# DoumanAsh/compu

Hardware: AMD Instinct MI355X
Metric: decompressed GB/s (whole node), batched 64 KiB DEFLATE blocks; % HBM peak (higher is better)
Workload: dtype u8

## Files before the change

compu_amd/csrc/inflate_unit.h:

```cpp
#pragma once
#include "chip_internal.h"
#include "wave_checksums.h"

namespace chip {

typedef uint32_t u32x2 __attribute__((ext_vector_type(2)));
typedef uint32_t u32x4 __attribute__((ext_vector_type(4)));
typedef u32x4 u32x4_u __attribute__((aligned(1)));
typedef u32x4 u32x4_a4 __attribute__((aligned(4)));
template <typename T>
__device__ __forceinline__ GAS T *rdfirst_gptr(T *p)
{
    return (GAS T *)rdfirst_ptr(p);
}

#ifndef CHIP_PHASE_FN
#define CHIP_PHASE_FN __attribute__((always_inline))
#endif

#ifdef CHIP_STATS
#define STAT_DECL unsigned long long st_[24] = {0}; unsigned long long st_t0_ = 0
#define STAT_T0() (st_t0_ = __builtin_readcyclecounter())
#define STAT_ACC(i) do { unsigned long long n_ = __builtin_readcyclecounter(); st_[i] += n_ - st_t0_; st_t0_ = n_; } while (0)
#define STAT_ADD(i, v) (st_[i] += (unsigned long long)(v))
#define STAT_PARAM , unsigned long long *st_, unsigned long long &st_t0_
#define STAT_ARG , st_, st_t0_
#else
#define STAT_DECL
#define STAT_T0()
#define STAT_ACC(i)
#define STAT_ADD(i, v)
#define STAT_PARAM
#define STAT_ARG
#endif

enum : uint32_t { K_LIT = 0, K_LEN = 1, K_EOB = 2, K_BAD = 3 };
__device__ __forceinline__ constexpr uint32_t mk_entry(uint32_t cl, uint32_t eb, uint32_t kind, uint32_t base)
{
    return cl | (eb << 4) | (kind << 8) | (base << 16);
}

constexpr int LIT_ROOT = 9;
constexpr int DIST_ROOT = 8;
constexpr int CL_ROOT = 7;

constexpr uint32_t F_HALT = 1u << 15, F_INV = 1u << 26, F_LEN = 1u << 31;
constexpr uint32_t D_BAD = 1u << 10, D_LONG = 1u << 15;
static_assert(15 - LIT_ROOT < 8 && 15 - DIST_ROOT < 8, "a root entry's index bit count leaves its bits [4:3] clear");
static_assert((2u << (15 - DIST_ROOT)) - 2u < 256u, "the distance sub-tables fit the 256 units that a root entry's offset spans");

__device__ __forceinline__ uint32_t make_final(uint32_t sym, uint32_t len)
{
    if (sym < 256) return len | (len << 10) | (sym << 16);
    if (sym == 256) return len | (len << 10) | F_HALT;
    if (sym >= 286) return len | (len << 10) | F_HALT | F_INV;
    const uint32_t s = sym - 257;
    uint32_t eb = 0, base = 3 + s;
    if (s == 28) base = 258;
    else if (s >= 8) {
        eb = (s >> 2) - 1;
        base = 3 + ((4 + (s & 3)) << eb);
    }
    return len | (eb << 5) | ((len + eb) << 10) | ((512u | base) << 16) | F_LEN;
}
__device__ __forceinline__ uint32_t make_dist16(uint32_t sym, uint32_t len)
{
    if (sym >= 30) return len | D_BAD;
    if (sym < 4) return len | (sym << 8);
    return len | (((sym >> 1) - 1) << 4) | ((2 + (sym & 1)) << 8);
}

#ifndef CHIP_S_BITS
#define CHIP_S_BITS 320
#define CHIP_XT_BITS 1536
#define CHIP_XT_BITS_FIXED 3072
#define CHIP_ROW_TOKENS 256
#endif
constexpr uint32_t S_BITS = CHIP_S_BITS;
constexpr uint32_t XT_BITS = CHIP_XT_BITS;
#ifndef CHIP_XT_BITS_FIXED
#define CHIP_XT_BITS_FIXED CHIP_XT_BITS
#endif
constexpr uint32_t XT_BITS_FIXED = CHIP_XT_BITS_FIXED;
constexpr uint32_t ROW_TOKENS = CHIP_ROW_TOKENS;
static_assert(S_BITS % 32 == 0 && ROW_TOKENS % 4 == 0 && 64 * ROW_TOKENS < 65536, "geometry");
constexpr uint32_t SEG_WORDS = S_BITS / 32 + 1;
constexpr uint32_t SEG_SHIFT = 24;
constexpr uint32_t SEG_MAGIC = ((1u << SEG_SHIFT) + S_BITS - 1) / S_BITS;
constexpr bool seg_magic_ok()
{
    for (uint32_t x = 0; x < 64u * S_BITS + 4096u; x++)
        if (((x * SEG_MAGIC) >> SEG_SHIFT) != x / S_BITS) return false;
    return true;
}
static_assert(seg_magic_ok() && (64u * S_BITS + 4096u) * (uint64_t)SEG_MAGIC < (1ull << 32), "segment index by multiplication");
constexpr uint32_t WIN_DW = (31 + 64 * S_BITS + 48 + 96 + 31) / 32 + 3;
constexpr uint32_t HDR_IN_DW = 192;

constexpr size_t ROWS_WORDS = (size_t)64 * ROW_TOKENS;
static_assert(64ull * ROW_TOKENS * 258 < (1ull << 32), "count_tokens() sums a super-round's output lengths in 32 bits");
__device__ __forceinline__ uint32_t row_base(uint32_t l) { return (l >> 3) * (8u * ROW_TOKENS) + (l & 7u) * 4u; }
__device__ __forceinline__ uint32_t row_word(uint32_t k) { return k + (k >> 2) * 28u; }

__device__ __forceinline__ uint32_t tok_olen(uint32_t t) { return (t & 512u) ? t & 0x1ffu : 1u + (t >> 31); }

struct HuffMeta {
    uint32_t limit15[16];
    uint32_t offs[16];
    uint32_t maxlen;
};

#ifndef CHIP_CHUNK_BYTES
#define CHIP_CHUNK_BYTES 2560
#endif
#ifndef CHIP_COPY_LANE_MAX
#define CHIP_COPY_LANE_MAX 32
#endif
constexpr uint32_t CHUNK_BYTES = CHIP_CHUNK_BYTES;
constexpr uint32_t COPY_LANE_MAX = CHIP_COPY_LANE_MAX;
constexpr uint32_t MQ_CAP = 128;
constexpr uint32_t IMG_WORDS = CHUNK_BYTES / 4 + 8;
constexpr uint32_t TOK_RING = 4;
static_assert(CHUNK_BYTES % 4 == 0 && CHUNK_BYTES >= 1024 && COPY_LANE_MAX % 16 == 0 && IMG_WORDS % 2 == 0, "geometry");

constexpr uint32_t FLUSH_BYTES = 4 * (IMG_WORDS + 2 * MQ_CAP + 64 * TOK_RING + 128 + 4);
constexpr uint32_t HDR_BYTES = 4 * HDR_IN_DW + 4 * (1 << CL_ROOT) + 80 + sizeof(HuffMeta) + 64 + 320 + 2 * 288 + 2 * 32 + 2 * sizeof(HuffMeta);
constexpr uint32_t PHASE_BYTES = 8 * WIN_DW > FLUSH_BYTES ? (8 * WIN_DW > HDR_BYTES ? 8 * WIN_DW : HDR_BYTES) : (FLUSH_BYTES > HDR_BYTES ? FLUSH_BYTES : HDR_BYTES);
#ifndef CHIP_LDS_BYTES
#define CHIP_LDS_BYTES 8960
#endif
constexpr uint32_t POOL_WORDS = (CHIP_LDS_BYTES - 2 * 512 - 2 * 256 - PHASE_BYTES) / 4;
constexpr uint32_t POOL_U16 = 2 * POOL_WORDS;
constexpr uint32_t DIST_SUB_BYTES = 2 * (POOL_U16 - 256);

struct alignas(16) WaveLds {
    union {
        struct {
            uint32_t win[WIN_DW];
            uint32_t bm[WIN_DW];
        } w;
        struct {
            uint32_t inbuf[HDR_IN_DW];
            uint32_t cl_lut[1 << CL_ROOT];
            uint32_t cl_sorted[20];
            HuffMeta cl_h;
            uint32_t count[16];
            uint8_t lens[320];
            uint16_t lit_sorted[288];
            uint16_t dist_sorted[32];
            HuffMeta lit_h, dist_h;
        } hdr;
        struct {
            uint32_t out[IMG_WORDS];
            uint2 mq[MQ_CAP];
            uint32_t tok[64 * TOK_RING];
            uint32_t pk[128];
            uint32_t trash[4];
        } fl;
        uint32_t phase_words_[PHASE_BYTES / 4];
    };
    uint16_t lit_root[1 << LIT_ROOT];
    uint16_t dist_root[1 << DIST_ROOT];
    uint32_t pool[POOL_WORDS];
};
static_assert(sizeof(WaveLds) <= CHIP_LDS_BYTES, "the waves per CU that CHIP_LDS_BYTES stands for");
static_assert(POOL_WORDS >= 413 + 142, "the tables of any valid block fit");
#ifndef CHIP_EXP_ALLOW_SMALL_LDS
static_assert(sizeof(WaveLds) >= 2048 * 4, "wave_crc32 needs 8 KB");
#endif

__device__ __forceinline__ uint32_t canon_index(const HuffMeta &H, uint32_t x15, uint32_t &l)
{
    l = 1;
    if (x15 >= H.limit15[15]) return 0xffffffffu;
#pragma unroll
    for (int j = 1; j < 15; j++) l += (x15 >= H.limit15[j]) ? 1u : 0u;
    return H.offs[l] + ((x15 - H.limit15[l - 1]) >> (15 - l));
}

struct CanonLim {
    uint32_t lim[16];
};
__device__ __forceinline__ CanonLim canon_limits(const HuffMeta &H)
{
    CanonLim c;
#pragma unroll
    for (int j = 0; j < 16; j++) c.lim[j] = rdfirst(H.limit15[j]);
    return c;
}
template <int LO, int HI>
__device__ __forceinline__ uint32_t canon_index_in(const HuffMeta &H, const CanonLim &c, uint32_t x15, uint32_t &l)
{
    l = LO;
#pragma unroll
    for (int j = LO; j < HI; j++) l += (x15 >= c.lim[j]) ? 1u : 0u;
    return H.offs[l] + ((x15 - H.limit15[l - 1]) >> (15 - l));
}

template <typename SortedT, typename MakeT>
__device__ __forceinline__ int canon_prep(uint32_t *count, const uint8_t *lens, int n_, bool code_lengths, SortedT *sorted, HuffMeta &H, MakeT make)
{
    const uint32_t lane = lane_id();
    const int n = (int)rdfirst((uint32_t)n_);
    if (lane < 16) count[lane] = 0;
    WSYNC();
    for (int s = lane; s < n; s += 64) {
        uint32_t l = lens[s];
        if (l) atomicAdd(&count[l], 1u);
    }
    WSYNC();
    const uint32_t c = lane >= 1 && lane <= 15 ? count[lane] : 0u;
    const uint32_t cincl = wave_incl_scan(c);
    const uint32_t off = cincl - c;
    const uint32_t lim = wave_incl_scan(lane <= 15 ? c << (15u - (lane & 15u)) : 0u);
    const uint32_t present = (uint32_t)__ballot(c != 0);
    const uint32_t maxlen = present ? 31u - (uint32_t)__clz((int)present) : 0u;
    const bool over = __any(lane <= 15 && lim > 32768u);
    const int left = rdlane(lim, 15) < 32768u ? 1 : 0;
    uint32_t mynext = off;
    if (lane <= 15) {
        H.limit15[lane] = lim;
        H.offs[lane] = off;
    }
    if (lane == 0) H.maxlen = maxlen;
    WSYNC();
    if (maxlen == 0) return 1;
    if (over) return -1;
    if (left > 0 && (code_lengths || maxlen != 1)) return -1;
    for (int base = 0; base < n; base += 64) {
        int s = base + (int)lane;
        uint32_t l = s < n ? lens[s] : 0;
        for (uint32_t pm = present & 0xfffeu; pm; pm &= pm - 1u) {
            const uint32_t ll = (uint32_t)__builtin_ctz(pm);
            uint64_t m = __ballot(l == ll);
            uint32_t bp = rdlane(mynext, ll);
            if (l == ll) sorted[bp + __popcll(m & lanemask_lt())] = make((uint32_t)s, l);
            if (lane == ll) mynext += __popcll(m);
        }
    }
    WSYNC();
    return 0;
}

__device__ CHIP_PHASE_FN int build_cl_table(WaveLds &L)
{
    const uint32_t lane = lane_id();
    HuffMeta &H = L.hdr.cl_h;
    const int r = canon_prep(L.hdr.count, L.hdr.lens, 19, true, L.hdr.cl_sorted, H, [](uint32_t s, uint32_t l) { return mk_entry(l, 0, K_LIT, s); });
    if (r < 0) return -1;
    for (uint32_t idx = lane; idx < (1u << CL_ROOT); idx += 64) {
        uint32_t e = mk_entry(1, 0, K_LIT, 0);
        if (r == 0) {
            uint32_t l;
            const uint32_t ci = canon_index(H, __brev(idx) >> 17, l);
            e = ci == 0xffffffffu ? mk_entry(H.maxlen, 0, K_BAD, 0) : L.hdr.cl_sorted[ci];
        }
        L.hdr.cl_lut[idx] = e;
    }
    WSYNC();
    return 0;
}

__device__ CHIP_PHASE_FN int build_litlen(WaveLds &L, const uint8_t *lens, int n, uint32_t &used)
{
    const uint32_t lane = lane_id();
    HuffMeta &H = L.hdr.lit_h;
    uint16_t *const sorted = L.hdr.lit_sorted;
    const int r = canon_prep(L.hdr.count, lens, n, false, sorted, H, [](uint32_t s, uint32_t) { return (uint16_t)s; });
    if (r != 0) return -1;
    const CanonLim CL = canon_limits(H);
    const uint32_t lim_r = CL.lim[LIT_ROOT], top = CL.lim[15];
    const uint32_t nshort = rdfirst(H.offs[LIT_ROOT + 1 <= 15 ? LIT_ROOT + 1 : 15]);
    const uint32_t nsym = rdfirst(H.offs[15]) + rdfirst(L.hdr.count[15]);
    const uint32_t nfirst = rdfirst(H.maxlen) <= (uint32_t)LIT_ROOT ? nsym : nshort;
    if (nfirst + 1 > POOL_WORDS) return 1;
    for (uint32_t i = lane; i < nfirst; i += 64) {
        const uint32_t s = sorted[i];
        L.pool[i] = make_final(s, lens[s]);
    }
    const uint32_t bad_idx = nfirst;
    const uint32_t bad_e = rdfirst(H.maxlen) | (rdfirst(H.maxlen) << 10) | F_HALT | F_INV;
    if (lane == 0) L.pool[bad_idx] = bad_e;
    for (uint32_t idx = lane; idx < (1u << LIT_ROOT); idx += 64) {
        const uint32_t x15 = __brev(idx) >> 17;
        if (x15 >= top) L.lit_root[idx] = (uint16_t)(bad_idx << 5);
        else if (x15 < lim_r) {
            uint32_t l;
            L.lit_root[idx] = (uint16_t)(canon_index_in<1, LIT_ROOT>(H, CL, x15, l) << 5);
        }
    }
    used = nfirst + 1;
    if (top > lim_r) {
        constexpr uint32_t P = 1u << (15 - LIT_ROOT);
        const uint32_t np = (top - lim_r + P - 1) / P;
        for (uint32_t j0 = 0; j0 < np; j0 += 64) {
            const uint32_t j = j0 + lane;
            const bool have = j < np;
            const uint32_t xj = lim_r + j * P;
            uint32_t sb = 0;
            if (have) {
                uint32_t l;
                (void)canon_index_in<LIT_ROOT + 1, 15>(H, CL, xj + P < top ? xj + P - 1 : top - 1, l);
                sb = l - LIT_ROOT;
            }
            const uint32_t size = have ? (1u << sb) : 0u;
            const uint32_t incl = wave_incl_scan(size);
            const uint32_t off = used + incl - size;
            const uint32_t total = rdlane(incl, 63);
            if (used + total > POOL_WORDS) return 1;
            if (have) {
                for (uint32_t t = 0; t < size; t++) {
                    const uint32_t x15 = sb ? xj + ((__brev(t) >> (32 - sb)) << (15 - LIT_ROOT - sb)) : xj;
                    uint32_t l, e = bad_e;
                    if (x15 < top) {
                        const uint32_t s = sorted[canon_index_in<LIT_ROOT + 1, 15>(H, CL, x15, l)];
                        e = make_final(s, l);
                    }
                    L.pool[off + t] = e;
                }
                L.lit_root[__brev(xj >> (15 - LIT_ROOT)) >> (32 - LIT_ROOT)] = (uint16_t)((off << 5) | sb);
            }
            used += total;
        }
    }
    WSYNC();
    return 0;
}

__device__ CHIP_PHASE_FN int build_dist(WaveLds &L, const uint8_t *lens, int n, uint32_t used)
{
    const uint32_t lane = lane_id();
    HuffMeta &H = L.hdr.dist_h;
    uint16_t *const sorted = L.hdr.dist_sorted;
    const int r = canon_prep(L.hdr.count, lens, n, false, sorted, H, [](uint32_t s, uint32_t) { return (uint16_t)s; });
    if (r < 0) return -1;
    if (r == 1) {
        for (uint32_t idx = lane; idx < (1u << DIST_ROOT); idx += 64) L.dist_root[idx] = (uint16_t)(1u | D_BAD);
        WSYNC();
        return 0;
    }
    const CanonLim CL = canon_limits(H);
    const uint32_t lim_r = CL.lim[DIST_ROOT], top = CL.lim[15], maxlen = rdfirst(H.maxlen);
    uint16_t *const pool16 = (uint16_t *)L.pool;
    for (uint32_t idx = lane; idx < (1u << DIST_ROOT); idx += 64) {
        const uint32_t x15 = __brev(idx) >> 17;
        if (x15 >= top) L.dist_root[idx] = (uint16_t)(maxlen | D_BAD);
        else if (x15 < lim_r) {
            uint32_t l;
            const uint32_t s = sorted[canon_index_in<1, DIST_ROOT>(H, CL, x15, l)];
            L.dist_root[idx] = (uint16_t)make_dist16(s, l);
        }
    }
    if (top > lim_r) {
        constexpr uint32_t P = 1u << (15 - DIST_ROOT);
        const uint32_t np = (top - lim_r + P - 1) / P;
        uint32_t used16 = 0;
        for (uint32_t j0 = 0; j0 < np; j0 += 64) {
            const uint32_t j = j0 + lane;
            const bool have = j < np;
            const uint32_t xj = lim_r + j * P;
            uint32_t sb = 0;
            if (have) {
                uint32_t l;
                (void)canon_index_in<DIST_ROOT + 1, 15>(H, CL, xj + P < top ? xj + P - 1 : top - 1, l);
                sb = l - DIST_ROOT;
            }
            const uint32_t size = have ? (1u << sb) : 0u;
            const uint32_t incl = wave_incl_scan(size);
            const uint32_t total = rdlane(incl, 63);
            if (2 * used + used16 + total > POOL_U16) return 1;
            const uint32_t base16 = POOL_U16 - used16 - incl;
            if (have) {
                for (uint32_t t = 0; t < size; t++) {
                    const uint32_t x15 = sb ? xj + ((__brev(t) >> (32 - sb)) << (15 - DIST_ROOT - sb)) : xj;
                    uint32_t l, e = maxlen | D_BAD;
                    if (x15 < top) {
                        const uint32_t s = sorted[canon_index_in<DIST_ROOT + 1, 15>(H, CL, x15, l)];
                        e = make_dist16(s, l);
                    }
                    pool16[base16 + t] = (uint16_t)e;
                }
                L.dist_root[__brev(xj >> (15 - DIST_ROOT)) >> (32 - DIST_ROOT)] = (uint16_t)(D_LONG | sb | ((2u * base16 - DIST_SUB_BYTES) << 3));
            }
            used16 += total;
        }
    }
    WSYNC();
    return 0;
}
__device__ __forceinline__ uint32_t pool_at(const WaveLds &L, uint32_t r, uint32_t x)
{
    return *(const uint32_t *)((const uint8_t *)L.pool + ((r >> 3) + (__builtin_amdgcn_ubfe(x, LIT_ROOT, r) << 2)));
}
__device__ __forceinline__ uint32_t dist_sub_at(const WaveLds &L, uint32_t m, uint32_t x)
{
    return *(const uint16_t *)((const uint8_t *)L.pool + DIST_SUB_BYTES + (__builtin_amdgcn_ubfe(m, 3, 9) + (__builtin_amdgcn_ubfe(x, DIST_ROOT, m) << 1)));
}

struct InWin {
    const uint32_t *g32;
    uint32_t total_dw;
    uint32_t win0;
};


__device__ __forceinline__ void win_load(WaveLds &L, InWin &w, uint32_t dw_start)
{
    WSYNC();
    w.win0 = dw_start;
    constexpr uint32_t PER_LANE = (HDR_IN_DW + 63) / 64;
    uint32_t v[PER_LANE];
#pragma unroll
    for (uint32_t j = 0; j < PER_LANE; j++) {
        const uint32_t i = dw_start + 64u * j + lane_id();
        v[j] = i < w.total_dw ? w.g32[i] : 0u;
    }
#pragma unroll
    for (uint32_t j = 0; j < PER_LANE; j++) {
        const uint32_t k = 64u * j + lane_id();
        if (k < HDR_IN_DW) L.hdr.inbuf[k] = v[j];
    }
    WSYNC();
}

__device__ __forceinline__ void win_ensure(WaveLds &L, InWin &w, uint32_t pos, uint32_t span = 64)
{
    uint32_t d = pos >> 5;
    if (d < w.win0 || d + ((span + 62u) >> 5) + 1u > w.win0 + HDR_IN_DW) win_load(L, w, d);
}

__device__ __forceinline__ void win_bits(const WaveLds &L, const InWin &w, uint32_t pos, uint32_t &lo, uint32_t &hi)
{
    uint32_t D = (pos >> 5) - w.win0, sh = pos & 31;
    uint32_t d0 = L.hdr.inbuf[D], d1 = L.hdr.inbuf[D + 1], d2 = L.hdr.inbuf[D + 2];
    lo = __builtin_amdgcn_alignbit(d1, d0, sh);
    hi = __builtin_amdgcn_alignbit(d2, d1, sh);
}

__device__ __forceinline__ void win_bits_uniform(const WaveLds &L, const InWin &w, uint32_t pos, uint32_t &lo, uint32_t &hi)
{
    uint32_t l, h;
    win_bits(L, w, pos, l, h);
    lo = rdfirst(l);
    hi = rdfirst(h);
}

__device__ __forceinline__ uint32_t bfe(uint32_t v, uint32_t off, uint32_t width) { return __builtin_amdgcn_ubfe(v, off, width); }

__device__ int32_t parse_wrapper(LDS_AS uint32_t *tab, const uint8_t *gin, uint32_t avail, int32_t format, uint32_t &wrap, uint32_t &hdr)
{
    wrap = 0;
    hdr = 0;
    if (avail < 2) return CHIP_NEED_INPUT;
    const uint32_t b0 = gin[0], b1 = gin[1];
    const bool allow_gzip = format == CHIP_FMT_GZIP || format == CHIP_FMT_AUTO;
    const bool allow_zlib = format == CHIP_FMT_ZLIB || format == CHIP_FMT_AUTO;
    if (allow_gzip && b0 == 0x1f && b1 == 0x8b) {
        wrap = 2;
        if (avail < 4) return CHIP_NEED_INPUT;
        const uint32_t flg = gin[3];
        if (gin[2] != 8) return Z_DATA_ERROR;
        if (flg & 0xe0) return Z_DATA_ERROR;
        if (avail < 10) return CHIP_NEED_INPUT;
        uint32_t k = 10;
        if (flg & 4) {
            if (avail < k + 2) return CHIP_NEED_INPUT;
            uint32_t xlen = gin[k] | ((uint32_t)gin[k + 1] << 8);
            k += 2;
            if (avail - k < xlen) return CHIP_NEED_INPUT;
            k += xlen;
        }
        for (uint32_t bit = 8; bit <= 16; bit <<= 1) {
            if (!(flg & bit)) continue;
            for (;;) {
                uint32_t idx = k + lane_id();
                uint64_t z = __ballot(idx < avail && gin[idx] == 0);
                if (z) {
                    k += (uint32_t)__ffsll((long long)z);
                    break;
                }
                if (avail - k <= 64) return CHIP_NEED_INPUT;
                k += 64;
            }
        }
        if (flg & 2) {
            if (avail < k + 2) return CHIP_NEED_INPUT;
            uint32_t crc = wave_crc32(tab, gin, k);
            if ((crc & 0xffffu) != (gin[k] | ((uint32_t)gin[k + 1] << 8))) return Z_DATA_ERROR;
            k += 2;
        }
        hdr = k;
        return ST_RUNNING;
    }
    if (!allow_zlib) return Z_DATA_ERROR;
    if (((b0 << 8) | b1) % 31u) return Z_DATA_ERROR;
    if ((b0 & 15u) != 8) return Z_DATA_ERROR;
    if ((b0 >> 4) + 8 > 15) return Z_DATA_ERROR;
    wrap = 1;
    hdr = 2;
    if (b1 & 0x20) {
        if (avail < 6) return CHIP_NEED_INPUT;
        hdr = 6;
        return CHIP_NEED_DICT;
    }
    return ST_RUNNING;
}

struct __attribute__((packed)) U32u { uint32_t v; };
struct __attribute__((packed)) U16u { uint16_t v; };
struct __attribute__((packed)) U128u { uint32_t x, y, z, w; };
typedef LDS_AS uint8_t lds_u8;

__device__ void wave_copy_stored(uint8_t *gdst, const uint32_t *g32, uint32_t total_dw, uint32_t so, uint32_t n)
{
    const uint32_t lane = lane_id();
    const uint8_t *gsrc = (const uint8_t *)g32 + so;
    uint32_t head = (uint32_t)((16u - ((uintptr_t)gdst & 15u)) & 15u);
    if (head > n) head = n;
    if (lane < head) gdst[lane] = gsrc[lane];
    uint32_t done = head;
    const uint32_t body = (n - done) & ~15u;
    if (body) {
        uint4 *d16 = (uint4 *)(gdst + done);
        const U128u *s16 = (const U128u *)(gsrc + done);
        const uint32_t cnt = body >> 4;
        uint32_t i = lane;
#ifdef CHIP_STORED_NT_LD
#define CHIP_STORED_LD(p) __builtin_nontemporal_load(p)
#else
#define CHIP_STORED_LD(p) (*(p))
#endif
#ifndef CHIP_STORED_PLAIN_ST
#define CHIP_STORED_ST(v, p) __builtin_nontemporal_store(v, p)
#else
#define CHIP_STORED_ST(v, p) (*(p) = (v))
#endif
#ifndef CHIP_STORED_DEPTH
#define CHIP_STORED_DEPTH 2
#endif
        for (; i + 64u * (CHIP_STORED_DEPTH - 1) < cnt; i += 64u * CHIP_STORED_DEPTH) {
            u32x4 v[CHIP_STORED_DEPTH];
#pragma unroll
            for (int k = 0; k < CHIP_STORED_DEPTH; k++) v[k] = CHIP_STORED_LD((const u32x4_u *)(s16 + i + 64u * k));
#pragma unroll
            for (int k = 0; k < CHIP_STORED_DEPTH; k++) CHIP_STORED_ST(v[k], (u32x4 *)(d16 + i + 64u * k));
        }
        for (; i < cnt; i += 64u) {
            const U128u a = s16[i];
            d16[i] = make_uint4(a.x, a.y, a.z, a.w);
        }
        done += body;
    }
    const uint32_t tail = n - done;
    if (lane < tail) gdst[done + lane] = gsrc[done + lane];
    (void)total_dw;
}

__device__ __forceinline__ uint32_t small_mod(uint32_t off, uint32_t d)
{
    uint32_t q = (uint32_t)(((float)off + 0.5f) * __builtin_amdgcn_rcpf((float)d));
    return off - q * d;
}
struct ChunkLds {
    uint32_t *out;
    uint2 *mq;
    uint32_t *tok;
    lds_u8 *trash;
};

__device__ __forceinline__ ChunkLds chunk_lds(WaveLds &L)
{
    ChunkLds c;
    c.out = L.fl.out;
    c.mq = L.fl.mq;
    c.tok = L.fl.tok;
    c.trash = (lds_u8 *)L.fl.trash;
    return c;
}

__device__ __forceinline__ void lds_put(lds_u8 *d, lds_u8 *trash, const U128u &v, uint32_t n)
{
    ((LDS_AS U32u *)(n >= 4 ? d : trash))->v = v.x;
    ((LDS_AS U32u *)((n >= 8 ? d : trash) + 4))->v = v.y;
    ((LDS_AS U32u *)((n >= 12 ? d : trash) + 8))->v = v.z;
    ((LDS_AS U32u *)((n >= 16 ? d : trash) + 12))->v = v.w;
    const uint32_t w = n < 4 ? v.x : n < 8 ? v.y : n < 12 ? v.z : v.w;
    lds_u8 *const t = d + (n & 12u);
    const bool two = (n & 2u) != 0, one = (n & 1u) != 0;
    ((LDS_AS U16u *)(two ? t : trash))->v = (uint16_t)w;
    *(one ? (two ? t + 2 : t) : trash) = (uint8_t)(two ? w >> 16 : w);
}

__device__ __forceinline__ void copy_one_match(lds_u8 *img, const uint8_t *base, uint32_t mis, uint32_t x, uint32_t len, uint32_t dist)
{
    const uint32_t lane = lane_id();
    const int32_t sx = (int32_t)x - (int32_t)dist;
    for (uint32_t i = lane; i < len; i += 64) {
        const int32_t s = sx + (int32_t)(dist >= len ? i : small_mod(i, dist));
        uint8_t b = 0;
        if (s < (int32_t)mis) b = ((GAS const uint8_t *)base)[s];
        if (s >= (int32_t)mis) b = img[s];
        img[x + i] = b;
    }
    LSYNC();
}

struct Round {
    uint32_t x, len, dist;
    bool glob;
    U128u v0, v1;
};

__device__ __forceinline__ void round_issue(Round &r, const ChunkLds &C, const uint8_t *base, uint32_t mis, uint32_t qh, uint32_t nr,
                                            bool glob_ok)
{
    const uint32_t lane = lane_id();
    const bool act = lane < nr;
    const uint32_t qi = (qh + lane) & (MQ_CAP - 1u);
    const uint2 e = C.mq[qi];
    r.x = e.x;
    const uint32_t ld = act ? e.y : 0u;
    r.len = ld & 0xffffu;
    r.dist = ld >> 16;
    const int32_t sx = (int32_t)r.x - (int32_t)r.dist;
    r.glob = glob_ok && r.len != 0 && r.len <= COPY_LANE_MAX && sx + (int32_t)r.len <= (int32_t)mis;
    r.v0 = U128u{0, 0, 0, 0};
    r.v1 = U128u{0, 0, 0, 0};
#ifndef CHIP_EXP_NO_GLOB
    if (r.glob) {
        const u32x4_u t = *(GAS const u32x4_u *)(base + sx);
        r.v0 = U128u{t.x, t.y, t.z, t.w};
    }
#endif
#ifndef CHIP_EXP_NO_GLOB
    if (r.glob && r.len > 16u) {
        const u32x4_u t = *(GAS const u32x4_u *)(base + sx + 16);
        r.v1 = U128u{t.x, t.y, t.z, t.w};
    }
#endif
}

__device__ __forceinline__ void round_finish(const Round &r, const ChunkLds &C, const uint8_t *base, uint32_t mis STAT_PARAM)
{
    const uint32_t lane = lane_id();
    lds_u8 *const img = (lds_u8 *)C.out;
    const int32_t sx = (int32_t)r.x - (int32_t)r.dist;
    uint64_t pend = __ballot(r.len != 0);
    STAT_ADD(14, 1);
    while (pend) {
        const uint32_t f = (uint32_t)__ffsll((long long)pend) - 1u;
        const uint32_t wp = rdlane(r.x, f);
        const bool mine = (pend >> lane) & 1ull;
        const bool loc = sx >= (int32_t)mis && (uint32_t)sx + r.len <= wp;
        const bool ready = mine && r.len <= COPY_LANE_MAX && (r.glob || loc);
        const uint64_t rm = __ballot(ready);
        if (!((rm >> f) & 1ull)) {
            STAT_ADD(15, 1);
            copy_one_match(img, base, mis, wp, rdlane(r.len, f), rdlane(r.dist, f));
            pend &= pend - 1ull;
            continue;
        }
        STAT_ADD(12, 1);
        uint32_t rem = ready ? r.len : 0u;
#pragma unroll
        for (uint32_t it = 0; it < COPY_LANE_MAX / 16; it++) {
            if (it && !__any(rem != 0)) break;
            U128u v = it ? r.v1 : r.v0;
            if (rem && !r.glob) {
                const lds_u8 *sp = img + sx + (int32_t)(16u * it);
                v.x = ((const LDS_AS U32u *)sp)->v;
                v.y = ((const LDS_AS U32u *)(sp + 4))->v;
                v.z = ((const LDS_AS U32u *)(sp + 8))->v;
                v.w = ((const LDS_AS U32u *)(sp + 12))->v;
            }
            const uint32_t n = rem < 16u ? rem : 16u;
            lds_put(img + r.x + 16u * it, C.trash, v, n);
            rem -= n;
        }
        LSYNC();
        pend &= ~rm;
    }
}

__device__ __forceinline__ uint32_t lane_gather(uint32_t x, uint32_t src)
{
    return (uint32_t)__builtin_amdgcn_ds_bpermute((int)(src << 2), (int)x);
// ... 450 lines not shown
    const uint32_t lane = lane_id();
    GAS const uint32_t *const grow = rdfirst_gptr(grow_);
    const uint32_t ntok = rdfirst(ntok_), npieces = rdfirst(npieces_);
    if (ntok == 0) return true;
    const bool have = lane < npieces;
    const uint32_t pfirst = have ? L.fl.pk[2u * lane] : ntok;
    const uint32_t pdelta = have ? L.fl.pk[2u * lane + 1u] : 0u;
    const uint32_t pnext = lane + 1u < npieces ? L.fl.pk[2u * lane + 2u] : ntok;
    const uint32_t k0 = (pfirst + pdelta) & 0xffffu;
    const uint32_t kend = k0 + (have ? pnext - pfirst : 0u);
    GAS const uint32_t *const row = grow + (pdelta >> 16);
    uint32_t sum = 0;
    for (uint32_t kq = k0 & ~3u; __any(kq < kend); kq += 4u) {
        if (kq < kend) {
            const u32x4 t = *(GAS const u32x4 *)(row + 8u * kq);
            const uint32_t t4[4] = {t.x, t.y, t.z, t.w};
#pragma unroll
            for (uint32_t j = 0; j < 4; j++)
                if (kq + j >= k0 && kq + j < kend) sum += tok_olen(t4[j]);
        }
    }
    const uint32_t incl = wave_incl_scan(sum);
    const uint32_t olo = rdfirst((uint32_t)osize), ohi = rdfirst((uint32_t)(osize >> 32));
    if (ohi == 0 && olo < 32768u) {
        uint32_t at = olo + incl - sum, badat = 0xffffffffu;
        for (uint32_t kq = k0 & ~3u; __any(kq < kend); kq += 4u) {
            if (kq < kend) {
                const u32x4 t = *(GAS const u32x4 *)(row + 8u * kq);
                const uint32_t t4[4] = {t.x, t.y, t.z, t.w};
#pragma unroll
                for (uint32_t j = 0; j < 4; j++)
                    if (kq + j >= k0 && kq + j < kend) {
                        const bool ismatch = (t4[j] & 512u) != 0;
                        if (ismatch && __builtin_amdgcn_ubfe(t4[j], 10, 16) + 1u > at && badat == 0xffffffffu) badat = at;
                        at += tok_olen(t4[j]);
                    }
            }
        }
        const uint64_t badm = __ballot(badat != 0xffffffffu);
        if (badm) {
            osize = rdlane(badat, (uint32_t)__ffsll((long long)badm) - 1u);
            status = Z_DATA_ERROR;
            return false;
        }
    }
    osize = (((uint64_t)ohi << 32) | olo) + rdlane(incl, 63u);
    return true;
}

template <bool SIZES>
__device__ CHIP_PHASE_FN void decode_block(WaveLds &L, InWin &w, uint32_t &pos, const uint32_t end_bit, uint8_t *gout, uint32_t &opos,
                                           const uint32_t cap, int32_t &status, uint32_t *rows, const uint32_t xt_bits, const uint32_t eob_len,
                                           const uint32_t flags, uint64_t &osize STAT_PARAM)
{
    pos = rdfirst(pos);
    opos = rdfirst(opos);
    for (;;) {
        if (pos >= end_bit) {
            status = CHIP_NEED_INPUT;
            return;
        }
        STAT_T0();
        uint32_t ntok = 0, why = 0, tpos = 0;
        const uint32_t npk = walk_round(L, w, pos, end_bit, rows, xt_bits, ntok, why, tpos STAT_ARG);
        int32_t st2 = ST_RUNNING;
        bool flushed = true;
        uint32_t ovf[3] = {0, 0, 0};
#ifdef CHIP_EXP_NO_FLUSH
        asm volatile("" ::"s"(npk), "s"(ntok));
#else
        if constexpr (SIZES) {
            if (npk) flushed = count_tokens(L, rows, ntok, npk, osize, st2);
        } else {
            if (npk) flushed = flush_tokens(L, rows, ntok, npk, gout, opos, cap, st2, ovf STAT_ARG);
        }
#endif
        w.win0 = 0xffffffffu;
        STAT_ACC(20);
        if (!flushed) {
            status = st2;
            if (!SIZES && (flags & F_COMPU_STATUS) && st2 == CHIP_NEED_OUTPUT) pos = overflow_bit(L, w, rows, ntok, npk, ovf[0], ovf[1], ovf[2], pos);
            return;
        }
        if (why == R_NEED_INPUT) {
            status = CHIP_NEED_INPUT;
            return;
        }
        if (why == R_EOB) {
            pos = tpos + eob_len;
            return;
        }
        if (why != R_LIMIT || tpos <= pos) {
            status = Z_DATA_ERROR;
            return;
        }
        pos = tpos;
    }
}

#ifndef CHIP_WAVES_PER_SIMD
#define CHIP_WAVES_PER_SIMD 5
#endif
#ifndef CHIP_INFLATE_MEMBERS
#define CHIP_INFLATE_MEMBERS 0
#endif
#ifndef CHIP_INFLATE_INDEX
#define CHIP_INFLATE_INDEX 0
#endif
#if CHIP_INFLATE_INDEX
struct IndexRec {
    uint64_t *pt_bit, *pt_out;
    uint64_t max_points;
    uint32_t spacing;
    uint32_t *walk;
};
#define INDEX_PARAM , const IndexRec &ix
#else
#define INDEX_PARAM
#endif
template <bool SIZES>
__device__ __attribute__((always_inline)) void inflate_unit(const BatchArgs &a, const uint32_t u, WaveLds &L, uint32_t *scratch, uint64_t *out_size INDEX_PARAM)
{
    const uint32_t lane = lane_id();

    const uint8_t *gin = a.in_base + a.in_off[u];
    const uint32_t in_len = a.in_len[u];
    uint8_t *gout = nullptr;
    uint32_t cap_ = 0xffffffffu;
    if constexpr (!SIZES) {
        gout = a.out_base + a.out_off[u];
        cap_ = a.out_cap[u];
    }
#if CHIP_INFLATE_MEMBERS
    uint32_t cap = cap_;
    uint32_t opos_members = 0;
    uint64_t osize_members = 0;
#else
    const uint32_t cap = cap_;
#endif
    uint64_t osize = 0;

    InWin w;
    const uint32_t mis = (uint32_t)((uintptr_t)gin & 3u);
    w.g32 = (const uint32_t *)(gin - mis);
    w.total_dw = (mis + in_len + 3u) >> 2;
    w.win0 = 0xffffffffu;
    const uint32_t start_bit = mis * 8u;
    const uint32_t end_bit = start_bit + in_len * 8u;

    uint32_t pos = start_bit;
    uint32_t opos = 0;
    int32_t status = ST_RUNNING;
    bool last = false;
    int tables = 0;
    uint32_t eob_len = 0;

    STAT_DECL;
    STAT_T0();
    uint32_t wrap = 0;
    int32_t format = a.format;
    uint32_t ck_bit = 0, ck_opos = 0;
    bool resumed = false;
    uint32_t run_check = 0, run_cov = 0, out_dropped = 0;
#if CHIP_INFLATE_INDEX
    uint32_t ix_n = 0, ix_out = 0, ix_end = 0;
#endif
    if (!SIZES && a.resume) {
        const uint32_t *rs = a.resume + RESUME_WORDS * u;
        const uint32_t r0 = rs[0], r1 = rs[1], r2 = rs[2];
        if (r0 != 0 && r0 <= in_len * 8u && r1 <= cap) {
            resumed = true;
            pos = start_bit + r0;
            opos = r1;
            wrap = r2 & 3u;
            ck_bit = r0;
            ck_opos = r1;
            run_check = rs[3];
            run_cov = rs[4];
            out_dropped = rs[5];
        }
    }
#if CHIP_INFLATE_MEMBERS
next_member:
#endif
    if (!resumed && format != CHIP_FMT_DEFLATE) {
        uint32_t hdr = 0;
#if CHIP_INFLATE_MEMBERS
        const uint32_t k0 = (pos - start_bit) >> 3;
        status = parse_wrapper((LDS_AS uint32_t *)&L, gin + k0, in_len - k0, format, wrap, hdr);
#else
        status = parse_wrapper((LDS_AS uint32_t *)&L, gin, in_len, format, wrap, hdr);
#endif
        status = (int32_t)rdfirst((uint32_t)status);
        wrap = rdfirst(wrap);
        pos += rdfirst(hdr) * 8u;
    }
    if (status == ST_RUNNING) win_load(L, w, pos >> 5);

    __builtin_amdgcn_s_setprio(2);
    while (status == ST_RUNNING) {
        if (last) {
#if CHIP_INFLATE_INDEX
            ix_end = pos - start_bit;
#endif
            status = CHIP_FINISHED;
            break;
        }
        ck_bit = pos - start_bit;
        ck_opos = opos;
#if CHIP_INFLATE_INDEX
        if (ix_n == 0 || opos - ix_out >= ix.spacing) {
            if (lane == 0 && ix_n < ix.max_points) {
                ix.pt_bit[ix_n] = ck_bit;
                ix.pt_out[ix_n] = opos;
            }
            ix_out = opos;
            ix_n++;
        }
#endif
        win_ensure(L, w, pos);
        if (pos + 3 > end_bit) {
            status = CHIP_NEED_INPUT;
            break;
        }
        uint32_t lo, hi;
        win_bits_uniform(L, w, pos, lo, hi);
        last = lo & 1u;
        uint32_t type = (lo >> 1) & 3u;
        pos += 3;
        if (type == 0) {
            pos = (pos + 7u) & ~7u;
            if (pos + 32 > end_bit) {
                status = CHIP_NEED_INPUT;
                break;
            }
            win_ensure(L, w, pos);
            win_bits_uniform(L, w, pos, lo, hi);
            uint32_t blen = lo & 0xffffu, nlen = lo >> 16;
            if (blen != (nlen ^ 0xffffu)) {
                status = Z_DATA_ERROR;
                break;
            }
            pos += 32;
            uint32_t avail = (end_bit - pos) >> 3;
            uint32_t ncopy = blen < avail ? blen : avail;
            if constexpr (SIZES) {
                osize += ncopy;
            } else {
                uint32_t room = cap - opos;
                if (ncopy > room) ncopy = room;
                wave_copy_stored(gout + opos, w.g32, w.total_dw, pos >> 3, ncopy);
                opos += ncopy;
            }
            pos += ncopy * 8u;
            if (ncopy < blen) {
                status = ncopy == avail ? CHIP_NEED_INPUT : CHIP_NEED_OUTPUT;
                break;
            }
            continue;
        }
        if (type == 3) {
            status = Z_DATA_ERROR;
            break;
        }
        uint32_t nlen = 288, ndist = 32;
        bool build = true;
        if (type == 1) {
            if (tables != 1) {
                for (uint32_t s = lane; s < 320; s += 64) L.hdr.lens[s] = s < 144 ? 8 : s < 256 ? 9 : s < 280 ? 7 : s < 288 ? 8 : 5;
                WSYNC();
                tables = 1;
            } else build = false;
        } else {
            tables = 2;
            if (pos + 14 > end_bit) {
                status = CHIP_NEED_INPUT;
                break;
            }
            win_ensure(L, w, pos);
            win_bits_uniform(L, w, pos, lo, hi);
            nlen = (lo & 31u) + 257;
            ndist = ((lo >> 5) & 31u) + 1;
            const uint32_t ncode = ((lo >> 10) & 15u) + 4;
            pos += 14;
            if (nlen > 286 || ndist > 30) {
                status = Z_DATA_ERROR;
                break;
            }
            if (pos + 3 * ncode > end_bit) {
                status = CHIP_NEED_INPUT;
                break;
            }
            win_ensure(L, w, pos, 128);
            if (lane < 19) L.hdr.lens[lane] = 0;
            WSYNC();
            if (lane < ncode) {
                static const uint8_t order[19] = {16, 17, 18, 0, 8, 7, 9, 6, 10, 5, 11, 4, 12, 3, 13, 2, 14, 1, 15};
                uint32_t l2, h2;
                win_bits(L, w, pos + 3 * lane, l2, h2);
                L.hdr.lens[order[lane]] = (uint8_t)(l2 & 7u);
            }
            WSYNC();
            pos += 3 * ncode;
            if (build_cl_table(L)) {
                status = Z_DATA_ERROR;
                break;
            }
            uint32_t have = 0, total = nlen + ndist, prevlen = 0;
            win_ensure(L, w, pos, 316 * 14 + 160);
            for (uint32_t k = lane; k < 320; k += 64) L.hdr.lens[k] = 0;
            WSYNC();
            while (have < total) {
                const uint32_t bp = pos + lane;
                uint32_t lo, hi;
                win_bits(L, w, bp, lo, hi);
                const uint32_t e = L.hdr.cl_lut[lo & 127u];
                const uint32_t cl = e & 15u, sym = e >> 16;
                const uint32_t eb = sym < 16 ? 0u : sym == 16 ? 2u : sym == 17 ? 3u : 7u;
                const uint32_t tl = cl + eb;
                const uint32_t run = sym < 16 ? 1u : (sym == 18 ? 11u : 3u) + bfe(lo, cl, eb);
                const uint32_t nx = lane + tl;
                uint32_t nth = 0;
                {
                    uint32_t pw = nx < 64u ? nx : 64u;
#pragma unroll
                    for (int r = 0; r < 6; r++) {
                        const uint32_t g1 = lane_gather(pw, nth & 63u), g2 = lane_gather(pw, pw & 63u);
                        if ((lane >> r) & 1u) nth = nth < 64u ? g1 : 64u;
                        pw = pw < 64u ? g2 : 64u;
                    }
                }
                uint8_t *const onflag = (uint8_t *)L.hdr.count;
                if (lane < 16) L.hdr.count[lane] = 0;
                LSYNC();
                if (nth < 64u) onflag[nth] = 1;
                LSYNC();
                const bool on = onflag[lane] != 0;
                const uint32_t c = on ? run : 0u;
                const uint32_t incl = wave_incl_scan(c);
                const uint32_t start = have + incl - c;
                const bool need = on && start < total;
                uint32_t bad = 0;
                if (need && bp + tl > end_bit) bad = 1;
                else if (need && sym == 16 && start == 0) bad = 2;
                else if (need && sym >= 16 && start + run > total) bad = 2;
                const uint64_t badm = __ballot(bad != 0);
                const uint32_t fb = badm ? (uint32_t)__ffsll((long long)badm) - 1u : 64u;
                const bool ok = need && lane < fb;
                const uint32_t expl = sym < 16 ? sym : 0u;
                const uint32_t m = wave_incl_max_scan((ok && sym != 16) ? (((lane + 1u) << 8) | expl) : 0u);
                const uint32_t v = sym == 16 ? (m ? m & 0xffu : prevlen) : expl;
                if (ok && sym < 16) L.hdr.lens[start] = (uint8_t)sym;
                if (ok && sym == 16)
                    for (uint32_t j = 0; j < run; j++) L.hdr.lens[start + j] = (uint8_t)v;
                if (badm) {
                    status = rdlane(bad, fb) == 1 ? (int32_t)CHIP_NEED_INPUT : Z_DATA_ERROR;
                    break;
                }
                const uint64_t okm = __ballot(ok);
                const uint32_t lv = 63u - (uint32_t)__clzll((long long)okm);
                have = rdlane(start + run, lv);
                pos += lv + rdlane(tl, lv);
                prevlen = rdlane(v, lv);
            }
            if (status != ST_RUNNING) break;
            WSYNC();
            STAT_ACC(4);
            if (rdfirst(L.hdr.lens[256]) == 0) {
                status = Z_DATA_ERROR;
                break;
            }
        }
        if (build) {
            eob_len = rdfirst(L.hdr.lens[256]);
            uint32_t used = 0;
            const int r1 = build_litlen(L, L.hdr.lens, (int)nlen, used);
            const int r2 = r1 ? r1 : build_dist(L, L.hdr.lens + nlen, (int)ndist, used);
            if (r1 || r2) {
                status = Z_DATA_ERROR;
                break;
            }
            STAT_ACC(5);
        }
        STAT_ACC(0);
        __builtin_amdgcn_s_setprio(0);
        decode_block<SIZES>(L, w, pos, end_bit, gout, opos, cap, status, scratch, tables == 1 ? XT_BITS_FIXED : XT_BITS, eob_len, a.flags, osize STAT_ARG);
        __builtin_amdgcn_s_setprio(2);
        STAT_T0();
    }
    __builtin_amdgcn_s_setprio(0);
    STAT_ACC(0);
    if (SIZES && status == CHIP_FINISHED && wrap) {
        uint32_t k = (pos - start_bit + 7u) >> 3;
        if (wrap == 1) {
            if (in_len - k < 4) status = CHIP_NEED_INPUT;
            k += 4;
        } else {
            if (in_len - k < 8) status = CHIP_NEED_INPUT;
            else {
                uint32_t isize = gin[k + 4] | ((uint32_t)gin[k + 5] << 8) | ((uint32_t)gin[k + 6] << 16) | ((uint32_t)gin[k + 7] << 24);
                if (rdfirst(isize) != (uint32_t)osize) status = Z_DATA_ERROR;
            }
            k += 8;
        }
        pos = start_bit + k * 8u;
    }
    if (!SIZES && status == CHIP_FINISHED && wrap) {
        uint32_t k = (pos - start_bit + 7u) >> 3;
        uint32_t need = wrap == 2 ? 8u : 4u;
        if (in_len - k < need && wrap == 1) {
            status = CHIP_NEED_INPUT;
        } else if (wrap == 1) {
            uint32_t want = ((uint32_t)gin[k] << 24) | ((uint32_t)gin[k + 1] << 16) | ((uint32_t)gin[k + 2] << 8) | gin[k + 3];
            const uint32_t c0 = run_cov - out_dropped;
            if (rdfirst(wave_adler32(gout + c0, opos - c0, resumed ? run_check : 1u)) != rdfirst(want)) status = Z_DATA_ERROR;
            k += 4;
        } else if (in_len - k < 4) {
            status = CHIP_NEED_INPUT;
        } else {
            uint32_t want = gin[k] | ((uint32_t)gin[k + 1] << 8) | ((uint32_t)gin[k + 2] << 16) | ((uint32_t)gin[k + 3] << 24);
            const uint32_t c0 = run_cov - out_dropped;
            if (rdfirst(wave_crc32((LDS_AS uint32_t *)&L, gout + c0, opos - c0, resumed ? run_check : 0u)) != rdfirst(want)) status = Z_DATA_ERROR;
            else if (in_len - k < 8) status = CHIP_NEED_INPUT;
            else {
                uint32_t isize = gin[k + 4] | ((uint32_t)gin[k + 5] << 8) | ((uint32_t)gin[k + 6] << 16) | ((uint32_t)gin[k + 7] << 24);
                if (rdfirst(isize) != out_dropped + opos) status = Z_DATA_ERROR;
            }
            k += 8;
        }
        pos = start_bit + k * 8u;
    }
#if CHIP_INFLATE_MEMBERS
    if (status == CHIP_FINISHED && wrap == 2) {
        const uint32_t k = (pos - start_bit) >> 3;
        if (in_len - k >= 2 && rdfirst(gin[k]) == 0x1fu && rdfirst(gin[k + 1]) == 0x8bu) {
            WSYNC();
            if constexpr (SIZES) {
                osize_members += osize;
                osize = 0;
            } else {
                gout += opos;
                cap -= opos;
                opos_members += opos;
                opos = 0;
            }
            format = CHIP_FMT_GZIP;
            status = ST_RUNNING;
            last = false;
            tables = 0;
            w.win0 = 0xffffffffu;
            goto next_member;
        }
    }
    opos += opos_members;
    osize += osize_members;
#endif
    STAT_ACC(6);
#ifdef CHIP_STATS
    if (a.stats && lane == 0)
        for (int k = 0; k < 24; k++) a.stats[(size_t)u * 24 + k] = st_[k];
#endif
    if (!SIZES && a.resume) {
        const bool cont = status == CHIP_NEED_INPUT || status == CHIP_NEED_OUTPUT;
        uint32_t *rs = a.resume + RESUME_WORDS * u;
        if (!resumed) run_check = wrap == 1 ? 1u : 0u;
        const uint32_t c0 = run_cov - out_dropped;
        if (cont && wrap && ck_bit != 0 && ck_opos > c0) {
            run_check = wrap == 1 ? wave_adler32(gout + c0, ck_opos - c0, run_check) : wave_crc32((LDS_AS uint32_t *)&L, gout + c0, ck_opos - c0, run_check);
            run_cov = out_dropped + ck_opos;
        }
        if (lane == 0) {
            rs[0] = cont ? ck_bit : 0u;
            rs[1] = cont ? ck_opos : 0u;
            rs[2] = wrap;
            rs[3] = run_check;
            rs[4] = run_cov;
            rs[5] = out_dropped;
        }
    }
    uint32_t used = (pos - start_bit + 7u) >> 3;
    if (used > in_len) used = in_len;
    if (!SIZES && (a.flags & F_COMPU_STATUS)) {
        if (status == CHIP_NEED_OUTPUT && used == in_len) status = CHIP_NEED_INPUT;
        else if (status == CHIP_NEED_INPUT && in_len == 0) status = CHIP_NEED_OUTPUT;
    }
#if CHIP_INFLATE_INDEX
    if (lane == 0) {
        ix.walk[0] = ix_n;
        ix.walk[1] = status == CHIP_FINISHED ? ix_end : 0u;
        ix.walk[2] = wrap;
    }
#endif
    if (lane == 0) {
        if constexpr (SIZES) out_size[u] = osize;
        else a.out_len[u] = opos;
        a.in_used[u] = status == CHIP_NEED_INPUT ? in_len : used;
        a.status[u] = status;
    }
}

}
```

Before: 348.5.

## Parallelize Huffman table build: ballot-based counting sort and flat subtable fill

The per-length ballot loop in canonical sorting is replaced by a 4-bit match-any ballot that ranks each lane among lanes with equal code length, with per-length cursors kept in LDS. The per-lane serial subtable fill in litlen and dist builds is replaced by a flattened fill where every lane writes one entry, using a max-scan over head words to find its owning subtable. The CL table build now uses precomputed limits, and the lens zeroing is done a dword at a time. This targets divergent serial loops in dynamic-header processing, at the cost of extra LDS syncs and scans, and it reuses cl_lut as scratch space.

```diff
diff --git a/compu_amd/csrc/inflate_unit.h b/compu_amd/csrc/inflate_unit.h
--- a/compu_amd/csrc/inflate_unit.h
+++ b/compu_amd/csrc/inflate_unit.h
@@ -198,7 +198,7 @@
 }
 
 template <typename SortedT, typename MakeT>
-__device__ __forceinline__ int canon_prep(uint32_t *count, const uint8_t *lens, int n_, bool code_lengths, SortedT *sorted, HuffMeta &H, MakeT make)
+__device__ __forceinline__ int canon_prep(uint32_t *count, const uint8_t *lens, int n_, bool code_lengths, SortedT *sorted, HuffMeta &H, MakeT make STAT_PARAM)
 {
     const uint32_t lane = lane_id();
     const int n = (int)rdfirst((uint32_t)n_);
@@ -217,10 +217,10 @@
     const uint32_t maxlen = present ? 31u - (uint32_t)__clz((int)present) : 0u;
     const bool over = __any(lane <= 15 && lim > 32768u);
     const int left = rdlane(lim, 15) < 32768u ? 1 : 0;
-    uint32_t mynext = off;
     if (lane <= 15) {
         H.limit15[lane] = lim;
         H.offs[lane] = off;
+        count[lane] = off;
     }
     if (lane == 0) H.maxlen = maxlen;
     WSYNC();
@@ -228,32 +228,41 @@
     if (over) return -1;
     if (left > 0 && (code_lengths || maxlen != 1)) return -1;
     for (int base = 0; base < n; base += 64) {
-        int s = base + (int)lane;
-        uint32_t l = s < n ? lens[s] : 0;
-        for (uint32_t pm = present & 0xfffeu; pm; pm &= pm - 1u) {
-            const uint32_t ll = (uint32_t)__builtin_ctz(pm);
-            uint64_t m = __ballot(l == ll);
-            uint32_t bp = rdlane(mynext, ll);
-            if (l == ll) sorted[bp + __popcll(m & lanemask_lt())] = make((uint32_t)s, l);
-            if (lane == ll) mynext += __popcll(m);
-        }
+        STAT_ADD(19, 1);
+        const int s = base + (int)lane;
+        const uint32_t l = s < n ? lens[s] : 0;
+        uint64_t same = ~0ull;
+#pragma unroll
+        for (uint32_t b = 0; b < 4; b++) {
+            const bool bit = (l >> b) & 1u;
+            const uint64_t m = __ballot(bit);
+            same &= bit ? m : ~m;
+        }
+        const uint32_t rank = __builtin_amdgcn_mbcnt_hi((uint32_t)(same >> 32), __builtin_amdgcn_mbcnt_lo((uint32_t)same, 0u));
+        const uint32_t cnt = (uint32_t)__popcll(same);
+        const uint32_t at = count[l];
+        if (l) sorted[at + rank] = make((uint32_t)s, l);
+        if (l && rank + 1u == cnt) count[l] = at + cnt;
+        LSYNC();
     }
     WSYNC();
     return 0;
 }
 
-__device__ CHIP_PHASE_FN int build_cl_table(WaveLds &L)
+__device__ CHIP_PHASE_FN int build_cl_table(WaveLds &L STAT_PARAM)
 {
     const uint32_t lane = lane_id();
     HuffMeta &H = L.hdr.cl_h;
-    const int r = canon_prep(L.hdr.count, L.hdr.lens, 19, true, L.hdr.cl_sorted, H, [](uint32_t s, uint32_t l) { return mk_entry(l, 0, K_LIT, s); });
+    const int r = canon_prep(L.hdr.count, L.hdr.lens, 19, true, L.hdr.cl_sorted, H, [](uint32_t s, uint32_t l) { return mk_entry(l, 0, K_LIT, s); } STAT_ARG);
     if (r < 0) return -1;
+    const CanonLim CL = canon_limits(H);
     for (uint32_t idx = lane; idx < (1u << CL_ROOT); idx += 64) {
         uint32_t e = mk_entry(1, 0, K_LIT, 0);
         if (r == 0) {
             uint32_t l;
-            const uint32_t ci = canon_index(H, __brev(idx) >> 17, l);
-            e = ci == 0xffffffffu ? mk_entry(H.maxlen, 0, K_BAD, 0) : L.hdr.cl_sorted[ci];
+            const uint32_t x15 = __brev(idx) >> 17;
+            const uint32_t ci = canon_index_in<1, CL_ROOT>(H, CL, x15 < CL.lim[15] ? x15 : 0u, l);
+            e = x15 < CL.lim[15] ? L.hdr.cl_sorted[ci] : mk_entry(rdfirst(H.maxlen), 0, K_BAD, 0);
         }
         L.hdr.cl_lut[idx] = e;
     }
@@ -261,17 +270,35 @@
     return 0;
 }
 
-__device__ CHIP_PHASE_FN int build_litlen(WaveLds &L, const uint8_t *lens, int n, uint32_t &used)
+static_assert(POOL_U16 <= 0x2000u, "a head word holds a flat index in 13 bits");
+template <typename PutT>
+__device__ __forceinline__ void fill_flat(uint32_t *heads, bool have, uint32_t sb, uint32_t start, uint32_t total, PutT put)
+{
+    const uint32_t lane = lane_id();
+    const uint32_t end = have ? start + (1u << sb) : 0u;
+    const uint32_t head = ((lane + 1u) << 16) | (start << 3) | sb;
+    for (uint32_t f0 = 0; f0 < total; f0 += 64) {
+        heads[lane] = 0;
+        if (end > f0 && start < f0 + 64u) heads[start > f0 ? start - f0 : 0u] = head;
+        LSYNC();
+        const uint32_t h = wave_incl_max_scan(heads[lane]);
+        LSYNC();
+        const uint32_t f = f0 + lane;
+        if (f < total) put(f, (h >> 16) - 1u, f - ((h >> 3) & 0x1fffu), h & 7u);
+    }
+}
+
+__device__ CHIP_PHASE_FN int build_litlen(WaveLds &L, const uint8_t *lens, int n, uint32_t &used STAT_PARAM)
 {
     const uint32_t lane = lane_id();
     HuffMeta &H = L.hdr.lit_h;
     uint16_t *const sorted = L.hdr.lit_sorted;
-    const int r = canon_prep(L.hdr.count, lens, n, false, sorted, H, [](uint32_t s, uint32_t) { return (uint16_t)s; });
+    const int r = canon_prep(L.hdr.count, lens, n, false, sorted, H, [](uint32_t s, uint32_t) { return (uint16_t)s; } STAT_ARG);
     if (r != 0) return -1;
     const CanonLim CL = canon_limits(H);
     const uint32_t lim_r = CL.lim[LIT_ROOT], top = CL.lim[15];
     const uint32_t nshort = rdfirst(H.offs[LIT_ROOT + 1 <= 15 ? LIT_ROOT + 1 : 15]);
-    const uint32_t nsym = rdfirst(H.offs[15]) + rdfirst(L.hdr.count[15]);
+    const uint32_t nsym = rdfirst(L.hdr.count[15]);
     const uint32_t nfirst = rdfirst(H.maxlen) <= (uint32_t)LIT_ROOT ? nsym : nshort;
     if (nfirst + 1 > POOL_WORDS) return 1;
     for (uint32_t i = lane; i < nfirst; i += 64) {
@@ -308,18 +335,17 @@
             const uint32_t off = used + incl - size;
             const uint32_t total = rdlane(incl, 63);
             if (used + total > POOL_WORDS) return 1;
-            if (have) {
-                for (uint32_t t = 0; t < size; t++) {
-                    const uint32_t x15 = sb ? xj + ((__brev(t) >> (32 - sb)) << (15 - LIT_ROOT - sb)) : xj;
-                    uint32_t l, e = bad_e;
-                    if (x15 < top) {
-                        const uint32_t s = sorted[canon_index_in<LIT_ROOT + 1, 15>(H, CL, x15, l)];
-                        e = make_final(s, l);
-                    }
-                    L.pool[off + t] = e;
+            STAT_ADD(22, (total + 63u) / 64u);
+            if (have) L.lit_root[__brev(xj >> (15 - LIT_ROOT)) >> (32 - LIT_ROOT)] = (uint16_t)((off << 5) | sb);
+            fill_flat(L.hdr.cl_lut, have, sb, incl - size, total, [&](uint32_t f, uint32_t p, uint32_t t, uint32_t b) {
+                const uint32_t x15 = lim_r + (j0 + p) * P + ((__brev(t) >> (32 - b)) << (15 - LIT_ROOT - b));
+                uint32_t l, e = bad_e;
+                if (x15 < top) {
+                    const uint32_t s = sorted[canon_index_in<LIT_ROOT + 1, 15>(H, CL, x15, l)];
+                    e = make_final(s, l);
                 }
-                L.lit_root[__brev(xj >> (15 - LIT_ROOT)) >> (32 - LIT_ROOT)] = (uint16_t)((off << 5) | sb);
-            }
+                L.pool[used + f] = e;
+            });
             used += total;
         }
     }
@@ -327,12 +353,12 @@
     return 0;
 }
 
-__device__ CHIP_PHASE_FN int build_dist(WaveLds &L, const uint8_t *lens, int n, uint32_t used)
+__device__ CHIP_PHASE_FN int build_dist(WaveLds &L, const uint8_t *lens, int n, uint32_t used STAT_PARAM)
 {
     const uint32_t lane = lane_id();
     HuffMeta &H = L.hdr.dist_h;
     uint16_t *const sorted = L.hdr.dist_sorted;
-    const int r = canon_prep(L.hdr.count, lens, n, false, sorted, H, [](uint32_t s, uint32_t) { return (uint16_t)s; });
+    const int r = canon_prep(L.hdr.count, lens, n, false, sorted, H, [](uint32_t s, uint32_t) { return (uint16_t)s; } STAT_ARG);
     if (r < 0) return -1;
     if (r == 1) {
         for (uint32_t idx = lane; idx < (1u << DIST_ROOT); idx += 64) L.dist_root[idx] = (uint16_t)(1u | D_BAD);
@@ -369,19 +395,18 @@
             const uint32_t incl = wave_incl_scan(size);
             const uint32_t total = rdlane(incl, 63);
             if (2 * used + used16 + total > POOL_U16) return 1;
+            STAT_ADD(23, (total + 63u) / 64u);
             const uint32_t base16 = POOL_U16 - used16 - incl;
-            if (have) {
-                for (uint32_t t = 0; t < size; t++) {
-                    const uint32_t x15 = sb ? xj + ((__brev(t) >> (32 - sb)) << (15 - DIST_ROOT - sb)) : xj;
-                    uint32_t l, e = maxlen | D_BAD;
-                    if (x15 < top) {
-                        const uint32_t s = sorted[canon_index_in<DIST_ROOT + 1, 15>(H, CL, x15, l)];
-                        e = make_dist16(s, l);
-                    }
-                    pool16[base16 + t] = (uint16_t)e;
+            if (have) L.dist_root[__brev(xj >> (15 - DIST_ROOT)) >> (32 - DIST_ROOT)] = (uint16_t)(D_LONG | sb | ((2u * base16 - DIST_SUB_BYTES) << 3));
+            fill_flat(L.hdr.cl_lut, have, sb, incl - size, total, [&](uint32_t f, uint32_t p, uint32_t t, uint32_t b) {
+                const uint32_t x15 = lim_r + (j0 + p) * P + ((__brev(t) >> (32 - b)) << (15 - DIST_ROOT - b));
+                uint32_t l, e = maxlen | D_BAD;
+                if (x15 < top) {
+                    const uint32_t s = sorted[canon_index_in<DIST_ROOT + 1, 15>(H, CL, x15, l)];
+                    e = make_dist16(s, l);
                 }
-                L.dist_root[__brev(xj >> (15 - DIST_ROOT)) >> (32 - DIST_ROOT)] = (uint16_t)(D_LONG | sb | ((2u * base16 - DIST_SUB_BYTES) << 3));
-            }
+                pool16[POOL_U16 - used16 - (f - t) - (1u << b) + t] = (uint16_t)e;
+            });
             used16 += total;
         }
     }
@@ -1438,15 +1463,17 @@
             }
             WSYNC();
             pos += 3 * ncode;
-            if (build_cl_table(L)) {
+            if (build_cl_table(L STAT_ARG)) {
                 status = Z_DATA_ERROR;
                 break;
             }
             uint32_t have = 0, total = nlen + ndist, prevlen = 0;
             win_ensure(L, w, pos, 316 * 14 + 160);
-            for (uint32_t k = lane; k < 320; k += 64) L.hdr.lens[k] = 0;
+            static_assert(offsetof(WaveLds, hdr.lens) % 4 == 0 && sizeof(L.hdr.lens) == 320, "lens[] is zeroed a dword at a time");
+            for (uint32_t k = lane; k < 320 / 4; k += 64) ((uint32_t *)L.hdr.lens)[k] = 0;
             WSYNC();
             while (have < total) {
+                STAT_ADD(7, 1);
                 const uint32_t bp = pos + lane;
                 uint32_t lo, hi;
                 win_bits(L, w, bp, lo, hi);
@@ -1510,8 +1537,8 @@
         if (build) {
             eob_len = rdfirst(L.hdr.lens[256]);
             uint32_t used = 0;
-            const int r1 = build_litlen(L, L.hdr.lens, (int)nlen, used);
-            const int r2 = r1 ? r1 : build_dist(L, L.hdr.lens + nlen, (int)ndist, used);
+            const int r1 = build_litlen(L, L.hdr.lens, (int)nlen, used STAT_ARG);
+            const int r2 = r1 ? r1 : build_dist(L, L.hdr.lens + nlen, (int)ndist, used STAT_ARG);
             if (r1 || r2) {
                 status = Z_DATA_ERROR;
                 break;
```

New measurement: 357.0 (median of 6 runs). +2.5%, better.
